# nmonette/TO-UED

Measured on AMD Instinct MI355X. Metric: agent-env-steps/sec (inner rollout) at num_agents=512; meta-updates/sec, higher is better.
Workload: dtype f32; 1 GPU; C2 LPG meta-gradient env_mode=tabular num_agents=512 num_mini_batches=1 W=64 T=20 K=5 score_function=random; num_agents=512, agents_per_gpu=512, env_workers=64, train_rollout_len=20, num_agent_updates=5, parallelism=dp1 (agent axis)

## Files before the change

to-ued_amd/csrc/wgrad.hip:

```cpp
#include <stdlib.h>
#include "common.h"

typedef float floatx4 __attribute__((ext_vector_type(4)));
typedef unsigned u32x4 __attribute__((ext_vector_type(4)));


namespace {

TOUED_DEV floatx4 mfma16(float a, float b, floatx4 c) { return __builtin_amdgcn_mfma_f32_16x16x4f32(a, b, c, 0, 0, 0); }

TOUED_DEV float f4(const float4& v, int e) { return e == 0 ? v.x : e == 1 ? v.y : e == 2 ? v.z : v.w; }

template <int NRT>
__global__ void __launch_bounds__(512, 2) k_wgrad(const float* __restrict__ A, long lda, int ra,
                                                  const float* __restrict__ B, long ldb, int rb, long K, long kchunk,
                                                  float* __restrict__ part) {
  constexpr int RA = NRT * 16;
  __shared__ float4 As[2][RA * 8];
  const int tid = threadIdx.x, lane = tid & 63, g = lane >> 4, c16 = lane & 15;
  const int wave = __builtin_amdgcn_readfirstlane(tid >> 6);
  const int ct = blockIdx.x, sc = blockIdx.y;
  const long kb = (long)sc * kchunk;
  const long ke = kb + kchunk < K ? kb + kchunk : K;
  const int nslab = (int)((ke - kb) / 32);
// ... 60 lines not shown
TOUED_DEV floatx4 mfma_bf(bf16x8 a, bf16x8 b, floatx4 c) {
  return __builtin_amdgcn_mfma_f32_16x16x32_bf16(a, b, c, 0, 0, 0);
}

template <typename V>
TOUED_DEV void split3_bf16(float x, V& p0, V& p1, V& p2, int e) {
  const __bf16 h = (__bf16)x;
  const float r1 = x - (float)h;
  const __bf16 m = (__bf16)r1;
  p0[e] = h;
  p1[e] = m;
  p2[e] = (__bf16)(r1 - (float)m);
}

TOUED_DEV int x6_slot(int row, int oct) { return row * 4 + (oct ^ ((0x78 >> (2 * ((row >> 2) & 3))) & 3)); }

__global__ void __launch_bounds__(64 * X6_NW, 1) k_wgrad_x6(const float* __restrict__ A, long lda, int ra,
                                                             const float* __restrict__ B, long ldb, int rb, long K,
                                                             long kchunk, float* __restrict__ part) {
  constexpr int NT = 64 * X6_NW;
  const int G = gridDim.x, ncol = (rb + X6_CT - 1) / X6_CT;
  const int xcd = blockIdx.x & 7;
  const int L = xcd * (G >> 3) + (xcd < (G & 7) ? xcd : (G & 7)) + (blockIdx.x >> 3);
  static_assert(X6_NS == 9 && 2 * X6_BT <= 8, "schedule below: 9 staging rounds at tiles 8-16, B splits before");
  __shared__ bf16x8 As[2][3][X6_RA * 4];
  const int tid = threadIdx.x, lane = tid & 63, q16 = lane & 15, oct = lane >> 4;
  const int wave = __builtin_amdgcn_readfirstlane(tid >> 6);
  const int ct = L % ncol, sc = L / ncol;
  const long kb = (long)sc * kchunk;
  const long ke = kb + kchunk < K ? kb + kchunk : K;
  const int nslab = (int)((ke - kb) / 32);
  const float4* Bp[X6_BT];
  int brow[X6_BT];
#pragma unroll
  for (int t = 0; t < X6_BT; ++t) {
    brow[t] = ct * X6_CT + 16 * (X6_BT * wave + t) + q16;
    Bp[t] = reinterpret_cast<const float4*>(B + (long)(brow[t] < rb ? brow[t] : 0) * ldb + kb) + 2 * oct;
  }
  float4 ast[X6_NS];
  auto a_index = [&](int j) {
    const int i = tid + NT * j;
    return j < X6_NS - 1 || i < X6_AQ ? i : i - NT;
  };
  auto load_a = [&](int s) {
#pragma unroll
    for (int j = 0; j < X6_NS; ++j) {
      const int i = a_index(j);
      const int row = (i >> 3) < ra ? (i >> 3) : ra - 1;
      ast[j] = *reinterpret_cast<const float4*>(A + (long)row * lda + kb + 32L * s + 4 * (i & 7));
    }
  };
  auto write_a = [&](int buf, int j) {
    const int i = a_index(j);
    const int row = i >> 3, kq = i & 7;
    const int slot = x6_slot(row, kq >> 1);
    bf16x4 p[3];
#pragma unroll
    for (int e = 0; e < 4; ++e) split3_bf16(f4(ast[j], e), p[0], p[1], p[2], e);
#pragma unroll
    for (int pc = 0; pc < 3; ++pc) reinterpret_cast<bf16x4*>(&As[buf][pc][slot])[kq & 1] = p[pc];
  };
  float4 bq[X6_BT][2];
  auto issue_b = [&](int s) {
#pragma unroll
    for (int t = 0; t < X6_BT; ++t) { bq[t][0] = Bp[t][8 * s]; bq[t][1] = Bp[t][8 * s + 1]; }
  };
  auto split_b = [&](bf16x8 (&dst)[X6_BT][3], int t, int half) {
#pragma unroll
    for (int e = 0; e < 4; ++e) split3_bf16(f4(bq[t][half], e), dst[t][0], dst[t][1], dst[t][2], 4 * half + e);
  };
  floatx4 acc[17][X6_BT];
#pragma unroll
  for (int i = 0; i < 17; ++i)
#pragma unroll
    for (int t = 0; t < X6_BT; ++t) acc[i][t] = floatx4{0.0f, 0.0f, 0.0f, 0.0f};

  auto slab = [&](int s, bf16x8 (&bp)[X6_BT][3], bf16x8 (&bpn)[X6_BT][3]) {
    const int buf = s & 1;
    load_a(s + 1 < nslab ? s + 1 : s);
    const bf16x8* a0p = As[buf][0];
    const bf16x8* a1p = As[buf][1];
    const bf16x8* a2p = As[buf][2];
    bf16x8 a[3];
    {
      const int slot = x6_slot(q16, oct);
      a[0] = a0p[slot]; a[1] = a1p[slot]; a[2] = a2p[slot];
    }
#pragma unroll
    for (int i = 0; i < 17; ++i) {
      bf16x8 an[3];
      if (i + 1 < 17) {
        const int slot = x6_slot(16 * (i + 1) + q16, oct);
        an[0] = a0p[slot]; an[1] = a1p[slot]; an[2] = a2p[slot];
      }
#pragma unroll
      for (int t = 0; t < X6_BT; ++t) {
        floatx4 c = acc[i][t];
        c = mfma_bf(a[2], bp[t][0], c);
        c = mfma_bf(a[1], bp[t][1], c);
        c = mfma_bf(a[0], bp[t][2], c);
        c = mfma_bf(a[1], bp[t][0], c);
        c = mfma_bf(a[0], bp[t][1], c);
        c = mfma_bf(a[0], bp[t][0], c);
        acc[i][t] = c;
      }
      if (i < 2 * X6_BT) split_b(bpn, i >> 1, i & 1);
      if (i == 2 * X6_BT) issue_b(s + 2 < nslab ? s + 2 : nslab - 1);
      if (i >= 8) write_a(buf ^ 1, i - 8);
      if (i + 1 < 17) {
        __builtin_amdgcn_sched_group_barrier(0x100, 3, 0);
      }
#pragma unroll
      for (int m = 0; m < 6 * X6_BT; ++m) {
        __builtin_amdgcn_sched_group_barrier(0x008, 1, 0);
        __builtin_amdgcn_sched_group_barrier(0x002, 1, 0);
      }
      __builtin_amdgcn_sched_barrier(0);
      if (i + 1 < 17) { a[0] = an[0]; a[1] = an[1]; a[2] = an[2]; }
    }
    lds_barrier();
  };

  bf16x8 bpa[X6_BT][3], bpb[X6_BT][3];
  if (nslab > 0) {
    load_a(0);
    issue_b(0);
#pragma unroll
    for (int j = 0; j < X6_NS; ++j) write_a(0, j);
#pragma unroll
    for (int t = 0; t < X6_BT; ++t) { split_b(bpa, t, 0); split_b(bpa, t, 1); }
    issue_b(nslab > 1 ? 1 : 0);
  }
  __syncthreads();
  for (int s = 0; s < nslab; ++s) {
    slab(s, bpa, bpb);
#pragma unroll
    for (int t = 0; t < X6_BT; ++t)
#pragma unroll
      for (int pc = 0; pc < 3; ++pc) bpa[t][pc] = bpb[t][pc];
  }
  const int rbp = ncol * X6_CT;
  float* out = part + (long)sc * X6_RA * rbp;
#pragma unroll
  for (int t = 0; t < X6_BT; ++t)
#pragma unroll
    for (int i = 0; i < 17; ++i)
#pragma unroll
      for (int r = 0; r < 4; ++r) out[(long)(16 * i + 4 * oct + r) * rbp + brow[t]] = acc[i][t][r];
}

typedef _Float16 f16x8 __attribute__((ext_vector_type(8)));
typedef _Float16 f16x4 __attribute__((ext_vector_type(4)));

TOUED_DEV floatx4 mfma_h(f16x8 a, f16x8 b, floatx4 c) {
  return __builtin_amdgcn_mfma_f32_16x16x32_f16(a, b, c, 0, 0, 0);
}

template <typename V>
TOUED_DEV void split2_f16(float y, V& p0, V& p1, int e) {
  const _Float16 h = (_Float16)y;
  p0[e] = h;
  p1[e] = (_Float16)(y - (float)h);
}
template <typename V>
TOUED_DEV void split2_f16s(float x, float s, V& p0, V& p1, int e) {
  const _Float16 h = (_Float16)__builtin_fmaf(x, s, 0.0f);
  p0[e] = h;
  p1[e] = (_Float16)__builtin_fmaf(x, s, -(float)h);
}

TOUED_DEV int scale_exp_of(float mx) {
  if (!(mx > 0.0f) || !(mx <= 3.0e38f)) return 0;
  int e;
  frexpf(mx, &e);
  return min(126, max(-126, 14 - e));
}

__global__ void __launch_bounds__(256) k_wgrad_rowmax(const float* __restrict__ A, long lda, int r0, long K,
                                                      long kper, int* __restrict__ bits) {
  const int row = r0 + blockIdx.y;
  const long kb = (long)blockIdx.x * kper, ke = kb + kper < K ? kb + kper : K;
  const float* a = A + (long)row * lda;
  float m = 0.0f;
  for (long k = kb + threadIdx.x * 4; k < ke; k += 256 * 4) {
    const float4 v = *reinterpret_cast<const float4*>(a + k);
    m = fmaxf(m, fmaxf(fmaxf(fabsf(v.x), fabsf(v.y)), fmaxf(fabsf(v.z), fabsf(v.w))));
  }
#pragma unroll
  for (int o = 32; o > 0; o >>= 1) m = fmaxf(m, __shfl_xor(m, o, 64));
  if ((threadIdx.x & 63) == 0) atomicMax(&bits[blockIdx.y], __float_as_int(m));
}

#ifdef WG_STAMPS
__device__ unsigned long long g_wg_stamps[64 * 8 * 64 * 4];
#define WG_STAMP(s, ph)                                                                                 \
  do {                                                                                                  \
    if (blockIdx.x < 64 && lane == 0 && (s) < 64)                                                       \
      g_wg_stamps[((blockIdx.x * 8 + wave) * 64 + (s)) * 4 + (ph)] = __builtin_amdgcn_s_memtime();      \
  } while (0)
#else
#define WG_STAMP(s, ph) do {} while (0)
#endif

#ifdef H3_PLACE
__device__ unsigned long long g_h3_place[64 * 256 * 4];
__device__ unsigned int g_h3_launch;
#endif

#ifndef H3_B_AUX
#define H3_B_AUX 0
#endif
template <int NW, int BT, int LAY>
__global__ void __launch_bounds__(64 * NW, 1) k_wgrad_h3(const float* __restrict__ A, long lda, int ra,
                                                        int a_unit_rows, const int* __restrict__ rowmax_bits,
                                                        const float* __restrict__ B, long ldb, int rb,
                                                        const int8_t* __restrict__ colexp, long K, long kchunk,
                                                        float* __restrict__ part, int ntiles, int* __restrict__ qctr,
                                                        int* __restrict__ visits) {
  constexpr int NT = 64 * NW;
  constexpr int CT = 16 * BT * NW;
  constexpr bool BSL = (LAY & 2) != 0, ASL = (LAY & 1) != 0;
  static_assert(!BSL || CT == 256, "slab-block B: one 256-row block per column tile");
  constexpr int NS = (X6_AQ + NT - 1) / NT;
  static_assert(NS <= 17 && 2 * BT < 17 - NS, "side-work schedule: B splits, B issue, then the staging rounds");
  const int ncol = (rb + CT - 1) / CT;
#ifdef H3_PLACE
  const unsigned long long t_start = __builtin_amdgcn_s_memrealtime();
#endif
  __shared__ int s_slot;
  if (threadIdx.x == 0) {
    const int x = __builtin_amdgcn_s_getreg((3 << 11) | 20) & 7;
    const int nch = ntiles / ncol, per = nch >> 3, rem = nch & 7;
    int got = -1;
    for (int y = 0; y < 8 && got < 0; ++y) {
      const int q = (x + y) & 7;
      const int cnt = ncol * (per + (q < rem ? 1 : 0));
      if (cnt == 0) continue;
      const int old = atomicAdd(&qctr[q], y == 0 ? 1 : 1 << 16);
      const int f = old & 0xFFFF, b = old >> 16;
      if (f + b < cnt) got = ncol * (q * per + (q < rem ? q : rem)) + (y == 0 ? f : cnt - 1 - b);
    }
    s_slot = got;
    if (visits && got >= 0) atomicAdd(&visits[got], 1);
  }
  __syncthreads();
  const int L = s_slot;
  if (L < 0) return;
  __shared__ f16x8 As[2][2][X6_RA * 4];
  __shared__ float asc[X6_RA];
  __shared__ int cred[NW];
  const int tid = threadIdx.x, lane = tid & 63, q16 = lane & 15, oct = lane >> 4;
  const int wave = __builtin_amdgcn_readfirstlane(tid >> 6);
  const int ct = L % ncol, sc = L / ncol;
  const long kb = (long)sc * kchunk;
  const long ke = kb + kchunk < K ? kb + kchunk : K;
  const int nslab = (int)((ke - kb) / 32);
  int cm = 127;
  for (long m = kb + 16L * tid; m < ke; m += 16L * NT) {
    const int4 v = *reinterpret_cast<const int4*>(colexp + m);
    const int w4[4] = {v.x, v.y, v.z, v.w};
#pragma unroll
    for (int q = 0; q < 4; ++q)
#pragma unroll
      for (int b = 0; b < 4; ++b) cm = min(cm, (int)(int8_t)(w4[q] >> (8 * b)));
  }
#pragma unroll
  for (int o = 32; o > 0; o >>= 1) cm = min(cm, __shfl_xor(cm, o, 64));
  if (lane == 0) cred[wave] = cm;
  for (int i = tid; i < X6_RA; i += NT) {
    const int r = i < ra ? i : ra - 1;
    asc[i] = r < a_unit_rows ? 16384.0f : ldexpf(1.0f, scale_exp_of(__int_as_float(rowmax_bits[r - a_unit_rows])));
  }
  __syncthreads();
  int cexp = cred[0];
#pragma unroll
  for (int w = 1; w < NW; ++w) cexp = min(cexp, cred[w]);
  if (cexp == 127) cexp = 0;
  const float bsc = ldexpf(1.0f, cexp);
  __amdgpu_buffer_rsrc_t rsB[BT];
  unsigned boff[BT];
  int brow[BT];
#pragma unroll
  for (int t = 0; t < BT; ++t) {
    const int tb = ct * CT + 16 * (BT * wave + t);
    const int tbc = tb < rb ? tb : rb - 1;
    brow[t] = tb + q16;
    const int rr = brow[t] < rb ? brow[t] : rb - 1;
    if (BSL) {
      rsB[t] = __builtin_amdgcn_make_buffer_rsrc(const_cast<float*>(B + (long)ct * 256 * K + (kb >> 5) * 256 * 32), 0,
                                                 -1, 0x00020000);
      boff[t] = (unsigned)((rr - ct * 256) * 128 + 16 * oct);
    } else {
      rsB[t] = __builtin_amdgcn_make_buffer_rsrc(const_cast<float*>(B + (long)tbc * ldb + kb), 0, -1, 0x00020000);
      boff[t] = (unsigned)(((long)(rr - tbc) * ldb + 4 * oct) * 4);
    }
  }
  float4 ast[NS];
  auto a_index = [&](int j) {
    const int i = tid + NT * j;
    return j < NS - 1 || i < X6_AQ ? i : X6_AQ - 8 + (i & 7);
  };
  const __amdgpu_buffer_rsrc_t rsA = __builtin_amdgcn_make_buffer_rsrc(const_cast<float*>(A), 0, -1, 0x00020000);
  constexpr int JS = ASL ? 2048 / NT : 0;
  static_assert(!ASL || (2048 % NT == 0 && JS <= NS - 1), "slab-block A: rounds split at row 256");
  const __amdgpu_buffer_rsrc_t rsAs =
      __builtin_amdgcn_make_buffer_rsrc(const_cast<float*>(A + (ASL ? (kb >> 5) * 256 * 32 : 0)), 0, -1, 0x00020000);
  unsigned avo[NS];
#pragma unroll
  for (int j = 0; j < NS; ++j) {
    const int i = a_index(j);
    const int row = (i >> 3) < ra ? (i >> 3) : ra - 1;
    avo[j] = j < JS ? (unsigned)((row * 32 + 4 * (i & 7)) * 4) : (unsigned)(((long)row * lda + 4 * (i & 7)) * 4);
  }
  auto load_a = [&](int s) {
#pragma unroll
    for (int j = 0; j < NS; ++j) {
      const u32x4 x = j < JS ? __builtin_amdgcn_raw_buffer_load_b128(rsAs, (int)avo[j], 32768 * s, 0)
                             : __builtin_amdgcn_raw_buffer_load_b128(rsA, (int)avo[j], (int)((kb + 32L * s) * 4), 0);
      ast[j] = make_float4(__uint_as_float(x.x), __uint_as_float(x.y), __uint_as_float(x.z), __uint_as_float(x.w));
    }
  };
  float asr[NS];
  auto write_a = [&](int buf, int j) {
    const int i = a_index(j);
    const int row = i >> 3, kq = i & 7;
    const int slot = x6_slot(row, kq & 3);
    const float s = asr[j];
    f16x4 p0, p1;
#pragma unroll
    for (int e = 0; e < 4; ++e) split2_f16s(f4(ast[j], e), s, p0, p1, e);
    reinterpret_cast<f16x4*>(&As[buf][0][slot])[kq >> 2] = p0;
    reinterpret_cast<f16x4*>(&As[buf][1][slot])[kq >> 2] = p1;
  };
  floatx4 acc[17][BT];
#pragma unroll
  for (int i = 0; i < 17; ++i)
#pragma unroll
    for (int t = 0; t < BT; ++t) acc[i][t] = floatx4{0.0f, 0.0f, 0.0f, 0.0f};

  float4 bq2[2][BT][2];
  auto issue_into = [&](float4 (&dst)[BT][2], int s) {
#pragma unroll
    for (int t = 0; t < BT; ++t)
#pragma unroll
      for (int hf = 0; hf < 2; ++hf) {
        const u32x4 x = __builtin_amdgcn_raw_buffer_load_b128(rsB[t], (int)boff[t], (BSL ? 32768 : 128) * s + 64 * hf,
                                                              H3_B_AUX);
        dst[t][hf] = make_float4(__uint_as_float(x.x), __uint_as_float(x.y), __uint_as_float(x.z), __uint_as_float(x.w));
      }
  };
  auto split_from = [&](const float4 (&src)[BT][2], f16x8 (&dst)[BT][2]) {
#pragma unroll
    for (int t = 0; t < BT; ++t)
#pragma unroll
      for (int hf = 0; hf < 2; ++hf)
#pragma unroll
        for (int e = 0; e < 4; ++e) split2_f16s(f4(src[t][hf], e), bsc, dst[t][0], dst[t][1], 4 * hf + e);
  };
  auto slab2 = [&](int s, f16x8 (&bp)[BT][2], const float4 (&nxt)[BT][2], float4 (&fill)[BT][2]) {
    WG_STAMP(s, 0);
    const int buf = s & 1;
    load_a(s + 1 < nslab ? s + 1 : s);
    const f16x8* a0p = As[buf][0];
    const f16x8* a1p = As[buf][1];
    constexpr int LA = NW == 4 ? 2 : 1;
    f16x8 fr[LA + 1][2];
#pragma unroll
    for (int d = 0; d < LA; ++d) {
      const int slot = x6_slot(16 * d + q16, oct);
      fr[d][0] = a0p[slot]; fr[d][1] = a1p[slot];
    }
#pragma unroll
    for (int i = 0; i < 17; ++i) {
      if (i + LA < 17) {
        const int slot = x6_slot(16 * (i + LA) + q16, oct);
        fr[(i + LA) % (LA + 1)][0] = a0p[slot]; fr[(i + LA) % (LA + 1)][1] = a1p[slot];
      }
      const f16x8(&a)[2] = fr[i % (LA + 1)];
#pragma unroll
      for (int t = 0; t < BT; ++t) {
        floatx4 c = acc[i][t];
        c = mfma_h(a[1], bp[t][0], c);
        c = mfma_h(a[0], bp[t][1], c);
        c = mfma_h(a[0], bp[t][0], c);
        acc[i][t] = c;
      }
      if (i == 1) issue_into(fill, s + 2 < nslab ? s + 2 : nslab - 1);
      if (i == 8) WG_STAMP(s, 1);
      if (i >= 17 - NS) write_a(buf ^ 1, i - (17 - NS));
      if (i == 16) split_from(nxt, bp);
      if (i + LA < 17) {
        __builtin_amdgcn_sched_group_barrier(0x100, 2, 0);
      }
#pragma unroll
      for (int m = 0; m < 3 * BT; ++m) {
        __builtin_amdgcn_sched_group_barrier(0x008, 1, 0);
        __builtin_amdgcn_sched_group_barrier(0x002, 3, 0);
      }
      __builtin_amdgcn_sched_barrier(0);
    }
    WG_STAMP(s, 2);
    lds_barrier();
    WG_STAMP(s, 3);
  };
#pragma unroll
  for (int j = 0; j < NS; ++j) asr[j] = asc[a_index(j) >> 3];
  f16x8 bpc[BT][2];
  if (nslab > 0) {
    load_a(0);
    issue_into(bq2[0], 0);
    issue_into(bq2[1], nslab > 1 ? 1 : 0);
#pragma unroll
    for (int j = 0; j < NS; ++j) write_a(0, j);
    split_from(bq2[0], bpc);
  }
  __syncthreads();
  int s2 = 0;
  for (; s2 + 1 < nslab; s2 += 2) {
    slab2(s2, bpc, bq2[1], bq2[0]);
    slab2(s2 + 1, bpc, bq2[0], bq2[1]);
  }
  if (s2 < nslab) slab2(s2, bpc, bq2[1], bq2[0]);
  const int rbp = ncol * CT;
  float* out = part + (long)sc * X6_RA * rbp;
  const float ib = ldexpf(1.0f, -cexp);
#pragma unroll
  for (int i = 0; i < 17; ++i)
#pragma unroll
    for (int r = 0; r < 4; ++r) {
      const float ia = 1.0f / asc[16 * i + 4 * oct + r];
#pragma unroll
      for (int t = 0; t < BT; ++t) out[(long)(16 * i + 4 * oct + r) * rbp + brow[t]] = (acc[i][t][r] * ia) * ib;
    }
#ifdef H3_PLACE
  __syncthreads();
  if (threadIdx.x == 0 && blockIdx.x < 256) {
    const unsigned slot = g_h3_launch & 63u;
    unsigned long long* e = g_h3_place + ((size_t)slot * 256 + blockIdx.x) * 4;
    e[0] = (unsigned long long)__builtin_amdgcn_s_getreg((3 << 11) | 20);
    e[1] = (unsigned long long)__builtin_amdgcn_s_getreg((31 << 11) | 4);
    e[2] = t_start;
    e[3] = __builtin_amdgcn_s_memrealtime();
  }
#endif
}

__global__ void k_wgrad_reduce(const float* __restrict__ part, int S, int RA, int rbp, int ra, int rb,
                               float* __restrict__ C, int ldc) {
  const long idx = (long)blockIdx.x * blockDim.x + threadIdx.x;
  if (idx >= (long)ra * rb) return;
  const int i = (int)(idx / rb), j = (int)(idx - (long)i * rb);
  float s = 0.0f;
  for (int c = 0; c < S; ++c) s += part[((long)c * RA + i) * rbp + j];
  C[(long)i * ldc + j] = s;
}

__global__ void k_wgrad_reduce_wave(const float* __restrict__ part, int S, int RA, int rbp, int ra, int rb,
                                    float* __restrict__ C, int ldc) {
  const long idx = ((long)blockIdx.x * blockDim.x + threadIdx.x) >> 6;
  const int lane = threadIdx.x & 63;
  if (idx >= (long)ra * rb) return;
  const int i = (int)(idx / rb), j = (int)(idx - (long)i * rb);
  float s = 0.0f;
  for (int c = lane; c < S; c += 64) s += part[((long)c * RA + i) * rbp + j];
#pragma unroll
  for (int m = 32; m >= 1; m >>= 1) s += __shfl_xor(s, m);
  if (lane == 0) C[(long)i * ldc + j] = s;
}

__global__ void __launch_bounds__(256) k_rowsum_part(const float* __restrict__ A, long lda, long K, long kchunk,
                                                     float* __restrict__ part) {
  const int c = blockIdx.x, i = blockIdx.y, ra = gridDim.y;
  const long kb = (long)c * kchunk, ke = kb + kchunk < K ? kb + kchunk : K;
  const float4* a4 = reinterpret_cast<const float4*>(A + (long)i * lda + kb);
  const long n4 = (ke - kb) / 4;
  float s = 0.0f;
  for (long m = threadIdx.x; m < n4; m += 256) {
    const float4 v = a4[m];
    s += (v.x + v.y) + (v.z + v.w);
  }
#pragma unroll
  for (int m = 32; m >= 1; m >>= 1) s += __shfl_xor(s, m);
  __shared__ float red[4];
  if ((threadIdx.x & 63) == 0) red[threadIdx.x >> 6] = s;
  __syncthreads();
  if (threadIdx.x == 0) part[(long)c * ra + i] = (red[0] + red[1]) + (red[2] + red[3]);
}

__global__ void k_rowsum_final(const float* __restrict__ part, int S, int ra, float* __restrict__ C, int ldc) {
  const int i = blockIdx.x, lane = threadIdx.x;
  float s = 0.0f;
  for (int c = lane; c < S; c += 64) s += part[(long)c * ra + i];
#pragma unroll
  for (int m = 32; m >= 1; m >>= 1) s += __shfl_xor(s, m);
  if (lane == 0) C[(long)i * ldc] = s;
}

struct Plan {
  int nrt, ncol, S, ct;
  bool x6;
  long kchunk;
};

static bool wgrad_f32_forced() {
  static const bool f = [] {
    const char* e = getenv("TOUED_WGRAD_F32");
    return e && e[0] == '1';
  }();
  return f;
}

static Plan plan(int ra, int rb, long K) {
  Plan p;
  p.nrt = ra <= 16 ? 1 : 17;
  p.x6 = p.nrt == 17 && !wgrad_f32_forced();
  p.ct = p.x6 ? X6_CT : 128;
  p.ncol = (rb + p.ct - 1) / p.ct;
  int cus = 256;
  int dev = 0;
  if (hipGetDevice(&dev) != hipSuccess ||
      hipDeviceGetAttribute(&cus, hipDeviceAttributeMultiprocessorCount, dev) != hipSuccess || cus < 1)
    cus = 256;
  {
    const int rsv = toued::current_ctx()->reserved_cus.load();
    cus = cus - rsv > cus / 2 ? cus - rsv : cus / 2;
  }
  int S = (p.x6 ? 1 : p.nrt == 1 ? 4 : 2) * cus / p.ncol;
  if (S < 1) S = 1;
  long slabs = K / 32;
  if (S > slabs) S = (int)(slabs > 0 ? slabs : 1);
  p.kchunk = ((slabs + S - 1) / S) * 32;
  p.S = (int)((K + p.kchunk - 1) / p.kchunk);
  if (p.S < 1) p.S = 1;
  return p;
}

}

extern "C" {

#ifdef H3_PLACE
int toued_dbg_h3_place(unsigned long long* host, unsigned* launches) {
  if (hipMemcpyFromSymbol(launches, HIP_SYMBOL(g_h3_launch), sizeof(unsigned)) != hipSuccess) return 1;
  return hipMemcpyFromSymbol(host, HIP_SYMBOL(g_h3_place), sizeof(g_h3_place)) == hipSuccess ? 0 : 1;
}
__global__ void k_h3_next() { if (threadIdx.x == 0) atomicAdd(&g_h3_launch, 1u); }
#endif
#ifdef WG_STAMPS
int toued_dbg_wgrad_stamps(unsigned long long* host) {
  return hipMemcpyFromSymbol(host, HIP_SYMBOL(g_wg_stamps), sizeof(g_wg_stamps)) == hipSuccess ? 0 : 1;
}
#endif

int toued_set_reserved_cus(int n) {
  return toued::current_ctx()->reserved_cus.exchange(n > 0 ? n : 0);
}

size_t toued_wgrad_workspace_floats(int ra, int rb, long K) {
  if (ra <= 0 || rb <= 0 || K <= 0) return 0;
  const Plan p = plan(ra, rb, K);
  return (size_t)p.S * p.nrt * 16 * p.ncol * p.ct;
}

static int wgrad_ldc(int ra, int rb, long K, const float* A, long lda, const float* B, long ldb, float* C, int ldc,
                     float* work, size_t work_floats, hipStream_t stream);

int toued_wgrad(int ra, int rb, long K, const float* A, long lda, const float* B, long ldb, float* C, float* work,
                size_t work_floats, hipStream_t stream) {
  return wgrad_ldc(ra, rb, K, A, lda, B, ldb, C, rb, work, work_floats, stream);
}

int toued_wgrad_ldc(int ra, int rb, long K, const float* A, long lda, const float* B, long ldb, float* C, int ldc,
                    float* work, size_t work_floats, hipStream_t stream) {
  return wgrad_ldc(ra, rb, K, A, lda, B, ldb, C, ldc, work, work_floats, stream);
}
// ... 199 lines not shown
```

to-ued_amd/toued/meta.py:

```python
from __future__ import annotations

import os
from dataclasses import dataclass

import torch

from . import _lib, prng
from .agents import AgentBatch
from .debug import nan_checker
from .lpg import LPGGRU, LPGLayout, Y
from .rollout import RolloutWrapper, Transition, split_rollouts


@dataclass
class LpgHyperparams:
    num_agent_updates: int = 5
    agent_target_coeff: float = 0.5
    policy_entropy_coeff: float = 5e-2
    target_entropy_coeff: float = 1e-3
    policy_l2_coeff: float = 5e-3
    target_l2_coeff: float = 1e-3
    gamma: float = 0.99
    gae_lambda: float = 0.95
    actor_lr: float = 40.0
# ... 230 lines not shown
        ptr = L.ptr
        L.call("toued_meta_keys", ptr(agent_keys), N, K, ptr(self.keys_roll), ptr(self.keys_eval),
               ptr(self.keys_ea_reset), ptr(self.keys_ea_roll), st)
        sparse = self.hist_sparse
        bound = not sparse and self.n_chunks == 1 and isinstance(agents, AgentBatch)
        ring = bound and os.environ.get("TOUED_HIST_RING", "1") != "0"
        r0 = self._ring if ring else 0
        if sparse:
            th = [agents.theta] * (K + 1)
            ph = [agents.phi] * (K + 1)
            self._live = (agents.theta, agents.phi)
        else:
            th = [self._theta_store[(r0 + k) % (K + 1)] for k in range(K + 1)]
            ph = [self._phi_store[(r0 + k) % (K + 1)] for k in range(K + 1)]
        self._ring_last = r0
        if sparse:
            if not (agents.theta.is_contiguous() and agents.phi.is_contiguous()):
                raise ValueError("MetaGradStep: the agents' tables must be contiguous (they are updated in place)")
        elif bound:
            if agents.theta.data_ptr() != th[0].data_ptr():
                th[0].copy_(agents.theta)
                ph[0].copy_(agents.phi)
                agents.theta = th[0]
                agents.phi = ph[0]
        else:
            th[0].copy_(agents.theta)
            ph[0].copy_(agents.phi)
        if not self.fused_step:
            self.G_th.zero_()
            self.G_ph.zero_()
        self.met.zero_()
        main = torch.cuda.current_stream()
        e1w, e1b = self._eta(eta, "e1_w"), self._eta(eta, "e1_b")
        e2w, e2b = self._eta(eta, "e2_w"), self._eta(eta, "e2_b")
        state = agents.state
        draws = None
        if split_rollouts():
            if self._draws is None:
                self._draws = tuple(torch.empty((T, (K + 1) * N * W, 4), dtype=torch.int32, device=self.dev)
                                    for _ in range(2))
            draws = self.ro.train_draws(self.keys_train, agents.levels, W,
                                        self._draws)
        ea = {}

        def start_eval_prep():
            self.side.wait_stream(main)
            with torch.cuda.stream(self.side):
                (_, _), ea["state"] = self.ro.batch_reset(self.keys_ea_reset, agents.levels, hyp.eval_workers)
                self._ea_draws = self.ro.eval_draws(self.keys_ea_roll, agents.levels, hyp.eval_workers,
                                                    self._ea_draws)
                ea["draws_done"] = torch.cuda.Event()
                ea["draws_done"].record(self.side)

        for k in range(K):
            tk = self._t(k)
            if self.fused_step and not sparse:
                self.side.wait_stream(main)
                with torch.cuda.stream(self.side):
                    th[k + 1].copy_(th[k])
                    ph[k + 1].copy_(ph[k])
                    copy_done = torch.cuda.Event()
                    copy_done.record(self.side)
            tok = self.timers.start("rollout")
            if draws is not None:
                self.ro.rollout_from_draws(draws, k, th[k], agents.levels, state, tk)
            else:
                self.ro.batch_rollout(self.keys_roll[k], th[k], agents.levels, state, out=tk,
                                      inplace_state=True)
            self.timers.stop(tok)
            nan_checker().check("rollout_rewards", tk.reward)
            L.call(lpg_inputs_fn(R, W), N, W, T, D, self.F, ptr(th[k]), ptr(ph[k]),
                   ptr(tk.obs_idx), ptr(tk.obs_time), ptr(tk.action), ptr(tk.reward), ptr(tk.done),
                   ptr(e1w), ptr(e1b), ptr(e2w), ptr(e2b), ptr(agents.step), ptr(agents.levels),
                   ptr(self.X) + 4 * k * T * R, self.gru.M, 1, 0, st)
            if k == 0:
                main.wait_event(self._packed)
            tok = self.timers.start("gru_fwd")
            self.gru.forward(k, self.X, tk.done, eta, self.pi_hat, self.y_hat)
            self.timers.stop(tok)
            if k == K - 1 and eval_keys_early() and eval_prep_after_forwards():
                start_eval_prep()
            if nan_checker().enabled:
                nan_checker().check("lpg_gru_states", self.gru.hin_block(k))
            nan_checker().check("lpg_outputs", self.pi_hat[k], self.y_hat[k])
            if sparse:
                L.call("toued_agent_step_snap", N, W, T, D, ptr(th[k]), ptr(ph[k]), ptr(tk.obs_idx), ptr(tk.obs_time),
                       ptr(tk.action), ptr(tk.reward), ptr(tk.done), ptr(self.pi_hat[k]), ptr(self.y_hat[k]),
                       hyp.agent_target_coeff, hyp.actor_lr, hyp.critic_lr, hyp.max_grad_norm, ptr(self.G_th[k]),
                       ptr(self.G_ph[k]), ptr(self.met[k]), ptr(agents.step), ptr(agents.levels), ptr(self.gstat[k]),
                       ptr(self.snap_th0[k]), ptr(self.snap_ph0[k]), ptr(self.snap_last0[k]), ptr(self.snap_th1[k]),
                       ptr(self.snap_ph1[k]), ptr(self.snap_last1[k]), st)
            elif self.fused_step:
                main.wait_event(copy_done)
                L.call("toued_agent_step_entropy" if self.step_entropy else "toued_agent_step", N, W, T, D,
                       ptr(th[k]), ptr(ph[k]), ptr(th[k + 1]), ptr(ph[k + 1]), ptr(tk.obs_idx), ptr(tk.obs_time),
                       ptr(tk.action), ptr(tk.reward), ptr(tk.done), ptr(self.pi_hat[k]), ptr(self.y_hat[k]),
                       hyp.agent_target_coeff, hyp.actor_lr, hyp.critic_lr, hyp.max_grad_norm, ptr(self.G_th[k]),
                       ptr(self.G_ph[k]), ptr(self.met[k]), ptr(agents.step), ptr(agents.levels), ptr(self.gstat[k]),
                       st)
                if not self.step_entropy:
                    L.call("toued_entropy", N, W, T, D, ptr(th[k + 1]), ptr(ph[k + 1]),
                           ptr(tk.obs_idx), ptr(tk.obs_time), ptr(self.met[k]), 0.0, 0.0, None, None, st)
            else:
                L.call("toued_agent_grad", N, W, T, D, ptr(th[k]), ptr(ph[k]), ptr(tk.obs_idx),
                       ptr(tk.obs_time), ptr(tk.action), ptr(tk.reward), ptr(tk.done), ptr(self.pi_hat[k]),
                       ptr(self.y_hat[k]), hyp.agent_target_coeff, ptr(self.G_th[k]), ptr(self.G_ph[k]),
                       ptr(self.met[k]), ptr(agents.step), ptr(agents.levels), ptr(self.gstat[k]), st)
                L.call("toued_agent_apply", N, D, ptr(th[k]), ptr(ph[k]), ptr(self.G_th[k]),
                       ptr(self.G_ph[k]), hyp.actor_lr, hyp.critic_lr, hyp.max_grad_norm, ptr(agents.step),
                       ptr(th[k + 1]), ptr(ph[k + 1]), ptr(self.gstat[k]), st)
                L.call("toued_entropy", N, W, T, D, ptr(th[k + 1]), ptr(ph[k + 1]),
                       ptr(tk.obs_idx), ptr(tk.obs_time), ptr(self.met[k]), 0.0, 0.0, None, None, st)
            nan_checker().check("agent_params", th[k + 1], ph[k + 1])
        if hyp.fix_value_critic:
            self.vc_loss.zero_()
            for k in range(K):
                self._value_critic_update(self._t(k), agents)
        te = self._t(K)
        if draws is not None:
            self.ro.rollout_from_draws(draws, K, th[K], agents.levels, state, te)
        else:
            self.ro.batch_rollout(self.keys_eval, th[K], agents.levels, state, out=te, inplace_state=True)
        L.call("toued_eval_loss", N, W, T, D, ptr(th[K]), ptr(agents.vcrit), ptr(te.obs_idx),
               ptr(te.obs_time), ptr(te.action), ptr(te.reward), ptr(te.done), hyp.gamma, hyp.gae_lambda,
               ptr(self.adv), ptr(self.abar), ptr(self.loss_out), st)
        if hyp.fix_value_critic:
            self._value_critic_update(te, agents)
        if not hyp.fix_value_critic:
            agents.vstep.add_(K + 1)
        key_cus = 2 * -(-N * hyp.eval_workers // 256)
        eval_cus = int(L.lib().toued_eval_returns_cus(N * hyp.eval_workers))

        def launch_eval():
            self.side.wait_stream(main)
            if "draws_done" not in ea:
                with torch.cuda.stream(self.side):
                    (_, _), ea["state"] = self.ro.batch_reset(self.keys_ea_reset, agents.levels, hyp.eval_workers)
                    self._ea_draws = self.ro.eval_draws(self.keys_ea_roll, agents.levels, hyp.eval_workers,
                                                        self._ea_draws)
                    ea["draws_done"] = torch.cuda.Event()
                    ea["draws_done"].record(self.side)
            ea["prev_reserve"] = L.lib().toued_set_reserved_cus(key_cus)

        def before_main_wgrad():
            small_done = torch.cuda.Event()
            small_done.record(main)
            self.side.wait_event(small_done)
            with torch.cuda.stream(self.side):
                ea["cum"] = self.ro.eval_returns_from_draws(self._ea_draws, th[K], agents.levels,
                                                            ea["state"])
            main.wait_event(ea["draws_done"])
            if os.environ.get("TOUED_EVAL_ALONE") == "1":
                main.wait_stream(self.side)
                return
            L.lib().toued_set_reserved_cus(eval_cus)
        if eval_keys_early() and "draws_done" not in ea:
            start_eval_prep()
        a_in = 0
        self.adj_th[a_in].zero_()
        self.adj_ph[a_in].zero_()
        L.call("toued_lpgloss_grad", N, W, T, D, ptr(th[K]), ptr(te.obs_idx), ptr(te.obs_time),
               ptr(te.action), ptr(self.abar), ptr(self.adj_th[a_in]), st)
        for k in range(K - 1, -1, -1):
            tk = self._t(k)
            if sparse:
                L.call("toued_entropy_clip_hvp_snap", N, W, T, D, K, ptr(self.snap_th1[k]), ptr(self.snap_ph1[k]),
                       ptr(self.snap_last1[k]), ptr(self.snap_th0[k]), ptr(self.snap_ph0[k]), ptr(self.snap_last0[k]),
                       ptr(tk.obs_idx), ptr(tk.obs_time), ptr(tk.action), ptr(self.pi_hat[k]), ptr(self.y_hat[k]),
                       -hyp.policy_entropy_coeff / K, -hyp.target_entropy_coeff / K, ptr(self.adj_th[a_in]),
                       ptr(self.adj_ph[a_in]), ptr(self.G_th[k]), ptr(self.G_ph[k]), ptr(self.gstat[k]), hyp.actor_lr,
                       hyp.critic_lr, hyp.max_grad_norm, ptr(self.coef), hyp.agent_target_coeff, hyp.policy_l2_coeff,
                       hyp.target_l2_coeff, ptr(self.d_pi_hat[k]), ptr(self.d_y_hat[k]), st)
                continue
            if self.fused_step and self.reverse_pair:
                L.call("toued_entropy_clip_hvp", N, W, T, D, K, ptr(th[k + 1]), ptr(ph[k + 1]),
                       ptr(th[k]), ptr(ph[k]), ptr(tk.obs_idx), ptr(tk.obs_time), ptr(tk.action),
                       ptr(self.pi_hat[k]), ptr(self.y_hat[k]), -hyp.policy_entropy_coeff / K,
                       -hyp.target_entropy_coeff / K, ptr(self.adj_th[a_in]), ptr(self.adj_ph[a_in]),
                       ptr(self.G_th[k]), ptr(self.G_ph[k]), ptr(self.gstat[k]), hyp.actor_lr, hyp.critic_lr,
                       hyp.max_grad_norm, ptr(self.coef), hyp.agent_target_coeff, hyp.policy_l2_coeff,
                       hyp.target_l2_coeff, ptr(self.d_pi_hat[k]), ptr(self.d_y_hat[k]), st)
                continue
            if self.fused_step:
                L.call("toued_entropy_clip", N, W, T, D, ptr(th[k + 1]), ptr(ph[k + 1]),
                       ptr(tk.obs_idx), ptr(tk.obs_time), -hyp.policy_entropy_coeff / K,
                       -hyp.target_entropy_coeff / K, ptr(self.adj_th[a_in]), ptr(self.adj_ph[a_in]),
                       ptr(self.G_th[k]), ptr(self.G_ph[k]), ptr(self.gstat[k]), hyp.actor_lr, hyp.critic_lr,
                       hyp.max_grad_norm, ptr(self.coef), st)
            else:
                L.call("toued_entropy", N, W, T, D, ptr(th[k + 1]), ptr(ph[k + 1]),
                       ptr(tk.obs_idx), ptr(tk.obs_time), None, -hyp.policy_entropy_coeff / K,
                       -hyp.target_entropy_coeff / K, ptr(self.adj_th[a_in]), ptr(self.adj_ph[a_in]), st)
                L.call("toued_clip_dot", N, D, ptr(self.G_th[k]), ptr(self.G_ph[k]), ptr(self.adj_th[a_in]),
                       ptr(self.adj_ph[a_in]), ptr(self.gstat[k]), hyp.actor_lr, hyp.critic_lr, hyp.max_grad_norm,
                       ptr(self.coef), st)
            L.call("toued_hvp", N, W, T, D, K, ptr(th[k]), ptr(ph[k]), ptr(tk.obs_idx),
                   ptr(tk.obs_time), ptr(tk.action), ptr(self.pi_hat[k]), ptr(self.y_hat[k]), ptr(self.G_th[k]),
                   ptr(self.G_ph[k]), ptr(self.adj_th[a_in]), ptr(self.adj_ph[a_in]), ptr(self.coef), hyp.actor_lr,
                   hyp.critic_lr, hyp.agent_target_coeff, hyp.policy_l2_coeff, hyp.target_l2_coeff,
                   ptr(self.adj_th[a_in]), ptr(self.adj_ph[a_in]), ptr(self.d_pi_hat[k]), ptr(self.d_y_hat[k]), st)
        try:
            self.gru.backward(self.traj.done, eta, self.y_hat, self.d_pi_hat, self.d_y_hat, self.X, self.grad,
                              self.timers, after_bwd=launch_eval,
                              before_main_wgrad=before_main_wgrad)
        finally:
            if "prev_reserve" in ea:
                L.lib().toued_set_reserved_cus(ea["prev_reserve"])
        if "cum" not in ea:
            raise RuntimeError("MetaGradStep: the GRU backward returned without launching eval_agent")
        tr = self.traj
        if sparse:
            L.call("toued_embed_bwd_snap", N, W, T, D, K, ptr(self.snap_ph0), ptr(self.snap_last0), ptr(tr.obs_time),
                   tr.obs_idx[0].numel(), ptr(tr.done), tr.done[0].numel(), ptr(self.gru.dX3), ptr(self.gru.dX4), T * R,
                   ptr(e1w), ptr(e1b), ptr(e2w), ptr(self.embed_partial), self.embed_blocks, st)
        else:
            L.call("toued_embed_bwd", N, W, T, D, K, ptr(self._phi_store), self._phi_store[0].numel(), r0,
                   ptr(tr.obs_idx), tr.obs_idx[0].numel(), ptr(tr.obs_time), ptr(tr.done), tr.done[0].numel(),
                   ptr(self.gru.dX3), ptr(self.gru.dX4), T * R, ptr(e1w), ptr(e1b), ptr(e2w), ptr(self.embed_partial),
                   self.embed_blocks, st)
        o = self.lay.offsets["e1_b"]
        assert self.lay.offsets["e2_w"] + 16 == o + 161
        L.call("toued_sum_rows_add", ptr(self.embed_partial), self.embed_blocks, 161, ptr(self.grad) + 4 * o, st)
        main.wait_stream(self.side)
        ea_cum = ea["cum"]
        ea_cum.record_stream(main)
        ea["state"].record_stream(main)
        nan_checker().check("eval_returns", ea_cum)
        if sparse:
            pass
        elif ring:
            agents.theta = th[K]
            agents.phi = ph[K]
            self._ring = (r0 + K) % (K + 1)
        else:
            agents.theta.copy_(th[K])
            agents.phi.copy_(ph[K])
        mo = torch.empty((6, N), dtype=torch.float32, device=self.dev)
        L.call("toued_meta_metrics", N, K, ptr(self.met), 1.0 / (W * T), ptr(self.loss_out),
               hyp.policy_entropy_coeff, hyp.policy_l2_coeff, hyp.target_entropy_coeff, hyp.target_l2_coeff, ptr(mo), st)
        return {
            "lpg_loss": self.loss_out[:, 0], "reg_lpg_loss": mo[0], "value_loss": self.loss_out[:, 1],
            "lpg_agent": {"policy_l2": mo[1], "policy_entropy": mo[2], "critic_loss": mo[3],
                          "critic_l2": mo[4], "critic_entropy": mo[5]},
            "lpg_agent_return": ea_cum.mean(dim=1),
        }

    def _value_critic_update(self, tk: Transition, agents):
        L = _lib
        L.call("toued_value_critic_update", self.N, self.W, self.T, self.D, L.ptr(agents.vcrit), L.ptr(tk.obs_idx),
               L.ptr(tk.obs_time), L.ptr(tk.reward), L.ptr(tk.done), self.hyp.gamma, self.hyp.gae_lambda,
               self.hyp.critic_lr, self.hyp.max_grad_norm, L.ptr(agents.vstep), L.ptr(self.vc_loss), L.stream_ptr())

    def _eval_rollout(self, keys, theta, levels, state):
        N = keys.shape[0]
        n = state.shape[1]
        cum = torch.empty((N, n // N), dtype=torch.float32, device=state.device)
        L = _lib
        L.call("toued_rollout", self.ro._c, L.ptr(levels), L.ptr(theta), theta.shape[1], L.ptr(keys), L.ptr(state),
               N, n // N, self.ro.eval_rollout_len, None, None, None, None, None, L.ptr(cum), L.stream_ptr())
        return cum


class AgentChunk:

    def __init__(self, agents, a0: int, a1: int, W: int):
        self._src = agents
        self._cols = (a0 * W, a1 * W)
        self.levels = agents.levels[a0:a1]
        self.theta = agents.theta[a0:a1]
        self.phi = agents.phi[a0:a1]
        self.step = agents.step[a0:a1]
        self.vcrit = None if agents.vcrit is None else agents.vcrit[a0:a1]
        self.vstep = None if agents.vstep is None else agents.vstep[a0:a1]
        self.state = agents.state[:, self._cols[0]:self._cols[1]].contiguous()

    @property
    def n(self) -> int:
        return self.levels.shape[0]

    def write_back(self):
        self._src.state[:, self._cols[0]:self._cols[1]].copy_(self.state)


def _map_metrics(m, fn):
    return {k: (_map_metrics(v, fn) if isinstance(v, dict) else fn(v)) for k, v in m.items()}


def _cat_metrics(parts):
    out = {}
    for k, v in parts[0].items():
        out[k] = _cat_metrics([p[k] for p in parts]) if isinstance(v, dict) else torch.cat([p[k] for p in parts])
    return out




@dataclass
class LpgTrainState:
    params: torch.Tensor
    opt: AdamState | None
    es: object | None = None

    @property
    def step(self) -> int:
        return self.opt.count if self.opt is not None else 0

# ... 63 lines not shown
```

Measured before the change: 183.7 million agent-env-steps/sec.

## Triple-buffer A staging in wgrad_h3 and move the LDS barrier mid-slab

Moves the f16 split of A from a double-buffered to a triple-buffered shared-memory scheme. Global loads and LDS writes for the next slab are interleaved across the first MFMA steps, and the per-slab LDS barrier moves from the end of the slab to a middle step. The first fragment reads of the following slab are prefetched across the slab boundary, and the slab loop is unrolled by a phase period so register rotation stays static. The aim is to hide barrier and staging latency behind MFMA work, at the cost of more LDS and a more complex schedule. It also restores the reserved-CU setting on the eval-alone debug path.

Measured after the change: 184.5 million agent-env-steps/sec (median of 6 runs). No clear change (+0.4%).

```diff
diff --git a/to-ued_amd/csrc/wgrad.hip b/to-ued_amd/csrc/wgrad.hip
--- a/to-ued_amd/csrc/wgrad.hip
+++ b/to-ued_amd/csrc/wgrad.hip
@@ -236,6 +236,9 @@
 typedef _Float16 f16x8 __attribute__((ext_vector_type(8)));
 typedef _Float16 f16x4 __attribute__((ext_vector_type(4)));
 
+template <int V>
+struct IntC { static constexpr int value = V; };
+
 TOUED_DEV floatx4 mfma_h(f16x8 a, f16x8 b, floatx4 c) {
   return __builtin_amdgcn_mfma_f32_16x16x32_f16(a, b, c, 0, 0, 0);
 }
@@ -306,7 +309,10 @@
   constexpr bool BSL = (LAY & 2) != 0, ASL = (LAY & 1) != 0;
   static_assert(!BSL || CT == 256, "slab-block B: one 256-row block per column tile");
   constexpr int NS = (X6_AQ + NT - 1) / NT;
-  static_assert(NS <= 17 && 2 * BT < 17 - NS, "side-work schedule: B splits, B issue, then the staging rounds");
+  constexpr int LA = NW == 4 ? 2 : 1;
+  constexpr int BAR = 8;
+  static_assert(NS < 16 && BAR >= NS - 1 && BAR < 17 - LA,
+                "side-work schedule: the staging rounds, B issue, the barrier, then the next slab's first reads");
   const int ncol = (rb + CT - 1) / CT;
 #ifdef H3_PLACE
   const unsigned long long t_start = __builtin_amdgcn_s_memrealtime();
@@ -328,9 +334,9 @@
     if (visits && got >= 0) atomicAdd(&visits[got], 1);
   }
   __syncthreads();
-  const int L = s_slot;
+  const int L = __builtin_amdgcn_readfirstlane(s_slot);
   if (L < 0) return;
-  __shared__ f16x8 As[2][2][X6_RA * 4];
+  __shared__ f16x8 As[3][2][X6_RA * 4];
   __shared__ float asc[X6_RA];
   __shared__ int cred[NW];
   const int tid = threadIdx.x, lane = tid & 63, q16 = lane & 15, oct = lane >> 4;
@@ -396,13 +402,10 @@
     const int row = (i >> 3) < ra ? (i >> 3) : ra - 1;
     avo[j] = j < JS ? (unsigned)((row * 32 + 4 * (i & 7)) * 4) : (unsigned)(((long)row * lda + 4 * (i & 7)) * 4);
   }
-  auto load_a = [&](int s) {
-#pragma unroll
-    for (int j = 0; j < NS; ++j) {
-      const u32x4 x = j < JS ? __builtin_amdgcn_raw_buffer_load_b128(rsAs, (int)avo[j], 32768 * s, 0)
-                             : __builtin_amdgcn_raw_buffer_load_b128(rsA, (int)avo[j], (int)((kb + 32L * s) * 4), 0);
-      ast[j] = make_float4(__uint_as_float(x.x), __uint_as_float(x.y), __uint_as_float(x.z), __uint_as_float(x.w));
-    }
+  auto load_a = [&](int j, int s) {
+    const u32x4 x = j < JS ? __builtin_amdgcn_raw_buffer_load_b128(rsAs, (int)avo[j], 32768 * s, 0)
+                           : __builtin_amdgcn_raw_buffer_load_b128(rsA, (int)avo[j], (int)((kb + 32L * s) * 4), 0);
+    ast[j] = make_float4(__uint_as_float(x.x), __uint_as_float(x.y), __uint_as_float(x.z), __uint_as_float(x.w));
   };
   float asr[NS];
   auto write_a = [&](int buf, int j) {
@@ -441,26 +444,24 @@
 #pragma unroll
         for (int e = 0; e < 4; ++e) split2_f16s(f4(src[t][hf], e), bsc, dst[t][0], dst[t][1], 4 * hf + e);
   };
-  auto slab2 = [&](int s, f16x8 (&bp)[BT][2], const float4 (&nxt)[BT][2], float4 (&fill)[BT][2]) {
+  f16x8 fr[LA + 1][2];
+  const int fslot = x6_slot(q16, oct);
+  auto slab3 = [&](auto ph, int s, int buf, f16x8 (&bp)[BT][2], const float4 (&nxt)[BT][2],
+                   float4 (&fill)[BT][2]) __attribute__((always_inline)) {
+    constexpr int P = decltype(ph)::value;
     WG_STAMP(s, 0);
-    const int buf = s & 1;
-    load_a(s + 1 < nslab ? s + 1 : s);
-    const f16x8* a0p = As[buf][0];
-    const f16x8* a1p = As[buf][1];
-    constexpr int LA = NW == 4 ? 2 : 1;
-    f16x8 fr[LA + 1][2];
-#pragma unroll
-    for (int d = 0; d < LA; ++d) {
-      const int slot = x6_slot(16 * d + q16, oct);
-      fr[d][0] = a0p[slot]; fr[d][1] = a1p[slot];
-    }
+    const int nbuf = buf == 2 ? 0 : buf + 1;
+    const int sn = s + 2 < nslab ? s + 2 : nslab - 1;
+    const f16x8* ap = &As[buf][0][fslot];
+    const f16x8* apn = &As[nbuf][0][fslot];
 #pragma unroll
     for (int i = 0; i < 17; ++i) {
-      if (i + LA < 17) {
-        const int slot = x6_slot(16 * (i + LA) + q16, oct);
-        fr[(i + LA) % (LA + 1)][0] = a0p[slot]; fr[(i + LA) % (LA + 1)][1] = a1p[slot];
-      }
-      const f16x8(&a)[2] = fr[i % (LA + 1)];
+      {
+        const int t = i + LA;
+        const f16x8* src = t < 17 ? ap + 64 * t : apn + 64 * (t - 17);
+        fr[(t + P) % (LA + 1)][0] = src[0]; fr[(t + P) % (LA + 1)][1] = src[X6_RA * 4];
+      }
+      const f16x8(&a)[2] = fr[(i + P) % (LA + 1)];
 #pragma unroll
       for (int t = 0; t < BT; ++t) {
         floatx4 c = acc[i][t];
@@ -469,42 +470,67 @@
         c = mfma_h(a[0], bp[t][0], c);
         acc[i][t] = c;
       }
-      if (i == 1) issue_into(fill, s + 2 < nslab ? s + 2 : nslab - 1);
+      if (i < NS) { write_a(nbuf, i); load_a(i, sn); }
+      if (i == NS) issue_into(fill, sn);
       if (i == 8) WG_STAMP(s, 1);
-      if (i >= 17 - NS) write_a(buf ^ 1, i - (17 - NS));
       if (i == 16) split_from(nxt, bp);
-      if (i + LA < 17) {
-        __builtin_amdgcn_sched_group_barrier(0x100, 2, 0);
-      }
+      __builtin_amdgcn_sched_group_barrier(0x100, 2, 0);
 #pragma unroll
       for (int m = 0; m < 3 * BT; ++m) {
         __builtin_amdgcn_sched_group_barrier(0x008, 1, 0);
         __builtin_amdgcn_sched_group_barrier(0x002, 3, 0);
       }
       __builtin_amdgcn_sched_barrier(0);
-    }
-    WG_STAMP(s, 2);
-    lds_barrier();
-    WG_STAMP(s, 3);
+      if (i == BAR) {
+        WG_STAMP(s, 2);
+        lds_barrier();
+        WG_STAMP(s, 3);
+      }
+    }
   };
 #pragma unroll
   for (int j = 0; j < NS; ++j) asr[j] = asc[a_index(j) >> 3];
   f16x8 bpc[BT][2];
   if (nslab > 0) {
-    load_a(0);
+#pragma unroll
+    for (int j = 0; j < NS; ++j) load_a(j, 0);
     issue_into(bq2[0], 0);
+#pragma unroll
+    for (int j = 0; j < NS; ++j) { write_a(0, j); load_a(j, nslab > 1 ? 1 : 0); }
     issue_into(bq2[1], nslab > 1 ? 1 : 0);
-#pragma unroll
-    for (int j = 0; j < NS; ++j) write_a(0, j);
     split_from(bq2[0], bpc);
   }
   __syncthreads();
-  int s2 = 0;
-  for (; s2 + 1 < nslab; s2 += 2) {
-    slab2(s2, bpc, bq2[1], bq2[0]);
-    slab2(s2 + 1, bpc, bq2[0], bq2[1]);
-  }
-  if (s2 < nslab) slab2(s2, bpc, bq2[1], bq2[0]);
+  if (nslab > 0) {
+#pragma unroll
+    for (int d = 0; d < LA; ++d) {
+      fr[d][0] = As[0][0][fslot + 64 * d]; fr[d][1] = As[0][1][fslot + 64 * d];
+    }
+    constexpr int R = LA + 1, PER = R % 2 == 0 ? R : 2 * R;
+    int s = 0, buf = 0;
+    auto one = [&](auto n) __attribute__((always_inline)) {
+      constexpr int N = decltype(n)::value;
+      if constexpr (N % 2 == 0) slab3(IntC<(17 * N) % R>{}, s, buf, bpc, bq2[1], bq2[0]);
+      else slab3(IntC<(17 * N) % R>{}, s, buf, bpc, bq2[0], bq2[1]);
+      buf = buf == 2 ? 0 : buf + 1;
+      return ++s < nslab;
+    };
+    while (s + PER <= nslab) {
+      one(IntC<0>{});
+      one(IntC<1>{});
+      if constexpr (PER == 6) {
+        one(IntC<2>{});
+        one(IntC<3>{});
+        one(IntC<4>{});
+        one(IntC<5>{});
+      }
+    }
+    if (s < nslab && one(IntC<0>{})) {
+      if constexpr (PER == 6) {
+        if (one(IntC<1>{}) && one(IntC<2>{}) && one(IntC<3>{})) one(IntC<4>{});
+      }
+    }
+  }
   const int rbp = ncol * CT;
   float* out = part + (long)sc * X6_RA * rbp;
   const float ib = ldexpf(1.0f, -cexp);
diff --git a/to-ued_amd/toued/meta.py b/to-ued_amd/toued/meta.py
--- a/to-ued_amd/toued/meta.py
+++ b/to-ued_amd/toued/meta.py
@@ -406,6 +406,7 @@
             main.wait_event(ea["draws_done"])
             if os.environ.get("TOUED_EVAL_ALONE") == "1":
                 main.wait_stream(self.side)
+                L.lib().toued_set_reserved_cus(ea["prev_reserve"])
                 return
             L.lib().toued_set_reserved_cus(eval_cus)
         if eval_keys_early() and "draws_done" not in ea:
```
